# 16lemoing/ccvs

Hardware: AMD Instinct MI355X
Metric: synthesized frames/sec (BAIR 256x256, cond=1, pred=15), whole job (higher is better)
Workload: dtype f32 (convolutions as split-bf16 x3 on bf16 MFMA, fp32 accumulate)

## Files before the change

ccvs_amd/csrc/conv2d_bf16.hip:

```cpp
#include "common.h"
#include "conv_common.h"
#include <stdlib.h>
#include <string.h>
#include <stdio.h>

#define CB_DECL(TWv, MBv) int ccvs_conv_bf16_launch_##TWv##_##MBv(const ConvK& k, const void* wsplit, const void* wktail, int CinG, int halo_h, int halo_w, int ntx_max, int gz, hipStream_t st, int wpc2);
CB_DECL(32, 4) CB_DECL(32, 2) CB_DECL(32, 1) CB_DECL(16, 4) CB_DECL(16, 2) CB_DECL(16, 1) CB_DECL(8, 4) CB_DECL(8, 2) CB_DECL(8, 1)
#undef CB_DECL

extern "C" int ccvs_conv_fetch_bytes_per_lane(const char* kernel_name) {
    if (!kernel_name) return -1;
    const char* pc = strstr(kernel_name, "conv2d_bf16x3_pc_kernel<");
    if (pc) {
        int tw = 0, mb = 0, nty = 0;
        if (sscanf(pc + strlen("conv2d_bf16x3_pc_kernel<"), " %d , %d , %d", &tw, &mb, &nty) != 3) return -1;
        const int b = conv_nty_fetch_bytes(nty);
        return b ? b : -1;
    }
    if (strstr(kernel_name, "conv2d_bf16x3_pt_kernel<")) return 16;
    if (strstr(kernel_name, "conv2d_bf16x3_kernel<") || strstr(kernel_name, "conv2d_mfma_kernel")) return 4;
    return -1;
}

static int g_conv_pt_mode = 1;
extern "C" int ccvs_conv_persistent_tiles(int32_t mode) {
    const int prev = __atomic_exchange_n(&g_conv_pt_mode, mode < 0 ? __atomic_load_n(&g_conv_pt_mode, __ATOMIC_RELAXED) : (int)(mode & 3), __ATOMIC_RELAXED);
    return prev;
}

extern "C" int ccvs_conv2d_bf16x3(const float* x, const void* w_split, const float* bias, const float* residual, float* y,
                                  const ccvs_conv_desc* d, void* stream) {
    CCVS_REQUIRE(x && w_split && y && d, "ccvs_conv2d_bf16x3: null pointer");
    CCVS_REQUIRE(d->N > 0 && d->Cin > 0 && d->Cout > 0 && d->Hin > 0 && d->Win > 0, "ccvs_conv2d_bf16x3: empty tensor");
    CCVS_REQUIRE((d->kh == d->kw || d->kw == 1 || d->kh == 1) && d->kh >= 1 && d->kh <= 9 && d->kw >= 1 && d->kw <= 9,
                 "ccvs_conv2d_bf16x3: kernel %dx%d unsupported", d->kh, d->kw);
    CCVS_REQUIRE(d->CoutPad % 32 == 0 && d->CoutPad >= d->Cout, "ccvs_conv2d_bf16x3: CoutPad %d invalid for Cout %d", d->CoutPad, d->Cout);
    int Hout, Wout;
    if (d->transposed) {
        CCVS_REQUIRE(d->kh == 3 && d->stride == 2 && d->pad == 0, "ccvs_conv2d_bf16x3: transposed supports k3 s2 p0 only");
        Hout = 2 * d->Hin + d->kh - 2;
        Wout = 2 * d->Win + d->kw - 2;
    } else {
        CCVS_REQUIRE(d->stride == 1 || d->stride == 2, "ccvs_conv2d_bf16x3: stride %d unsupported", d->stride);
        Hout = (d->Hin + 2 * d->pad - d->kh) / d->stride + 1;
        Wout = (d->Win + 2 * d->pad - d->kw) / d->stride + 1;
    }
    CCVS_REQUIRE(Hout == d->Hout && Wout == d->Wout, "ccvs_conv2d_bf16x3: output %dx%d expected, got %dx%d", Hout, Wout, d->Hout, d->Wout);

    ConvK k;
    k.x = x; k.w = nullptr; k.bias = bias; k.res = residual; k.y = y;
    k.N = d->N; k.Cin = d->Cin; k.Hin = d->Hin; k.Win = d->Win; k.in_sN = d->in_sN; k.in_sC = d->in_sC;
    k.Cout = d->Cout; k.CoutPad = d->CoutPad; k.Hout = d->Hout; k.Wout = d->Wout;
    k.out_sN = d->out_sN; k.out_sC = d->out_sC; k.res_sN = d->res_sN; k.res_sC = d->res_sC;
    k.kh = d->kh; k.kw = d->kw; k.stride = d->stride; k.pad = d->pad; k.transposed = d->transposed ? 1 : 0;
    k.act = d->act; k.accumulate = d->accumulate; k.out_scale = d->out_scale;
    k.pre = d->pre; k.pre_sN = d->pre_sN; k.pre_sC = d->pre_sC; k.pre_div = d->pre_div > 0 ? d->pre_div : 1;
    k.in_p8 = d->in_p8 ? 1 : 0; k.out_p8 = d->out_p8 ? 1 : 0;
    static const int pt_env = getenv_int("CCVS_CONV_PT", -1);
    k.pt = pt_env >= 0 ? pt_env : __atomic_load_n(&g_conv_pt_mode, __ATOMIC_RELAXED);
    k.ktail = 0; k.nwork = 0; k.gx = k.gy = 1; k.work0 = 0; k.xcd_chunk = 0; k.cu_limit = d->cu_limit > 0 ? d->cu_limit : ccvs_cu_limit_of(stream);
    k.zi = (d->pre && k.pre_div > 1 && !d->transposed && d->N % k.pre_div == 0) ? k.pre_div : 0;
    if (k.in_p8) CCVS_REQUIRE(!d->transposed && d->stride == 1 && d->Cin % 8 == 0, "ccvs_conv2d_bf16x3: packed input needs stride 1, Cin %% 8 == 0");
    if (k.out_p8) CCVS_REQUIRE(!d->transposed && d->Cout % 8 == 0 && !d->accumulate && !residual, "ccvs_conv2d_bf16x3: packed output needs Cout %% 8 == 0, no residual / accumulate");
    const int CinG = 2 * ((d->Cin + 15) / 16);

    const int VH = d->transposed ? (Hout + 1) / 2 : Hout;
    const int VW = d->transposed ? (Wout + 1) / 2 : Wout;
    const int TW = VW > 16 ? 32 : (VW > 8 ? 16 : 8);
    const int TH = 256 / TW;
    k.tiles_x = cdiv(VW, TW);
    k.tiles_y = cdiv(VH, TH);
    const int s = d->transposed ? 1 : d->stride;
    const int ext_y = d->transposed ? 1 : d->kh - 1, ext_x = d->transposed ? 1 : d->kw - 1;
    const int ntx_max = d->transposed ? 2 : d->kw;
    const int halo_h = (TH - 1) * s + ext_y + 1, halo_w = (TW - 1) * s + ext_x + 1;
    const int gz = d->N * (d->transposed ? 4 : 1);
    CCVS_REQUIRE(gz <= 65535, "ccvs_conv2d_bf16x3: batch %d too large for one launch", d->N);
    hipStream_t st = (hipStream_t)stream;
    int mb = (d->CoutPad % 128 == 0) ? 4 : ((d->CoutPad % 64 == 0) ? 2 : 1);
    constexpr long small_split = 256;
    while (mb > 1 && (long)k.tiles_x * k.tiles_y * gz * (d->CoutPad / (32 * mb)) < small_split) mb >>= 1;
    constexpr int wpc2_cin = 64;
    int wpc2 = 0;
    if (mb >= 2 && TW == 32 && d->Cin <= wpc2_cin && d->kh == 3 && d->kw == 3 && d->stride == 1 && !d->transposed && !d->in_p8 && !d->out_p8) {
        mb = 2;
        wpc2 = 1;
    }
#define CB_DISPATCH(TWv)                                                                                        \
    if (mb == 4) return ccvs_conv_bf16_launch_##TWv##_4(k, w_split, d->w_ktail, CinG, halo_h, halo_w, ntx_max, gz, st, wpc2);           \
    if (mb == 2) return ccvs_conv_bf16_launch_##TWv##_2(k, w_split, d->w_ktail, CinG, halo_h, halo_w, ntx_max, gz, st, wpc2);           \
    return ccvs_conv_bf16_launch_##TWv##_1(k, w_split, d->w_ktail, CinG, halo_h, halo_w, ntx_max, gz, st, wpc2);
    if (TW == 32) { CB_DISPATCH(32) }
    if (TW == 16) { CB_DISPATCH(16) }
    CB_DISPATCH(8)
#undef CB_DISPATCH
}
```

ccvs_amd/csrc/conv2d_bf16_core.h:

```cpp
#pragma once
#include "common.h"
#include "conv_common.h"

typedef __bf16 bf16x8 __attribute__((ext_vector_type(8)));
__device__ __forceinline__ void cb_store16(void* dst, f32x4 v) { *reinterpret_cast<f32x4*>(dst) = v; }
__device__ __forceinline__ void cb_store16(void* dst, uint4 v) { cb_store16(dst, f32x4{__uint_as_float(v.x), __uint_as_float(v.y), __uint_as_float(v.z), __uint_as_float(v.w)}); }

#define CB_NO_CLAMP(c) (c)
#define CB_LDS_BARRIER() asm volatile("s_waitcnt lgkmcnt(0)\n\ts_barrier" ::: "memory")

#define CB_TAP4_PRIME(OFF)                                                                                             \
    {                                                                                                                  \
        _Pragma("unroll") for (int pp = 0; pp < 4; ++pp) {                                                             \
            fq[pp][0] = __builtin_bit_cast(bf16x8, it0[OFF(0) + bofs[pp]]);                                            \
            fq[pp][1] = __builtin_bit_cast(bf16x8, it0[OFF(0) + plane + bofs[pp]]);                                    \
        }                                                                                                              \
        _Pragma("unroll") for (int m = 0; m < MB; ++m) {                                                               \
            fw[0][m][0] = __builtin_bit_cast(bf16x8, wt0[m * 32]);                                                     \
            fw[0][m][1] = __builtin_bit_cast(bf16x8, wt0[NT + m * 32]);                                                \
        }                                                                                                              \
    }
#define CB_TAP4(CUR, tb, more, OFF)                                                                                    \
    {                                                                                                                  \
        const uint4* itn_ = it0 + OFF((tb) + 1);                                                                       \
        if (more) {                                                                                                    \
            const uint4* wtn_ = wt0 + ((tb) + 1) * 4 * NT;                                                             \
            _Pragma("unroll") for (int m = 0; m < MB; ++m) {                                                           \
                fw[(CUR) ^ 1][m][0] = __builtin_bit_cast(bf16x8, wtn_[m * 32]);                                        \
                fw[(CUR) ^ 1][m][1] = __builtin_bit_cast(bf16x8, wtn_[NT + m * 32]);                                   \
            }                                                                                                          \
        }                                                                                                              \
        __builtin_amdgcn_sched_barrier(0);                                                                             \
        _Pragma("unroll") for (int m = 0; m < MB; ++m) {                                                               \
            _Pragma("unroll") for (int pp = 0; pp < 4; ++pp) {                                                         \
                acc[m][pp] = __builtin_amdgcn_mfma_f32_32x32x16_bf16(fw[CUR][m][1], fq[pp][0], acc[m][pp], 0, 0, 0);   \
                acc[m][pp] = __builtin_amdgcn_mfma_f32_32x32x16_bf16(fw[CUR][m][0], fq[pp][1], acc[m][pp], 0, 0, 0);   \
                acc[m][pp] = __builtin_amdgcn_mfma_f32_32x32x16_bf16(fw[CUR][m][0], fq[pp][0], acc[m][pp], 0, 0, 0);   \
                if (m == MB - 1 && (more)) {                                                                           \
                    fq[pp][0] = __builtin_bit_cast(bf16x8, itn_[bofs[pp]]);                                            \
                    fq[pp][1] = __builtin_bit_cast(bf16x8, itn_[plane + bofs[pp]]);                                    \
                }                                                                                                      \
            }                                                                                                          \
        }                                                                                                              \
    }

#define CB_LD_B(SET, tb, OFF)                                                                   \
    {                                                                                           \
        const uint4* it_ = it0 + OFF(tb);                                                       \
        _Pragma("unroll") for (int pp = 0; pp < 2; ++pp) {                                      \
            fb[SET][pp][0] = __builtin_bit_cast(bf16x8, it_[bofs[pp]]);                         \
            fb[SET][pp][1] = __builtin_bit_cast(bf16x8, it_[plane + bofs[pp]]);                 \
        }                                                                                       \
    }
#define CB_LD_A(SET, tb, m_)                                                                    \
    {                                                                                           \
        const uint4* wt_ = wt0 + (tb) * 4 * NT + (m_) * 32;                                     \
        fa[SET][0] = __builtin_bit_cast(bf16x8, wt_[0]);                                        \
        fa[SET][1] = __builtin_bit_cast(bf16x8, wt_[NT]);                                       \
    }
#define CB_TAP(BSET, A0, tb, has_next, OFF)                                                     \
    _Pragma("unroll") for (int m = 0; m < MB; ++m) {                                            \
        if (m + 1 < MB) {                                                                       \
            CB_LD_A(((A0) + m + 1) & 1, tb, m + 1)                                              \
        } else if (has_next) {                                                                  \
            CB_LD_A(((A0) + m + 1) & 1, (tb) + 1, 0)                                            \
            CB_LD_B((BSET) ^ 1, (tb) + 1, OFF)                                                  \
        }                                                                                       \
        __builtin_amdgcn_sched_barrier(0);  \
        _Pragma("unroll") for (int pp = 0; pp < 2; ++pp) {                                      \
            acc[m][pp] = __builtin_amdgcn_mfma_f32_32x32x16_bf16(fa[((A0) + m) & 1][1], fb[BSET][pp][0], acc[m][pp], 0, 0, 0); \
            acc[m][pp] = __builtin_amdgcn_mfma_f32_32x32x16_bf16(fa[((A0) + m) & 1][0], fb[BSET][pp][1], acc[m][pp], 0, 0, 0); \
            acc[m][pp] = __builtin_amdgcn_mfma_f32_32x32x16_bf16(fa[((A0) + m) & 1][0], fb[BSET][pp][0], acc[m][pp], 0, 0, 0); \
        }                                                                                       \
    }

#define CB_KTAIL(IH, WTL)                                                                                              \
    {                                                                                                                  \
        const int r_ = p.ktail, nq_ = 9 * r_, nj_ = (nq_ + 15) >> 4;                                                   \
        const unsigned short* ih = IH;                                                                                 \
        const uint4* wtl = WTL;                                                                                        \
        for (int j = 0; j < nj_; ++j) {                                                                                \
            bf16x8 gb[PP][2];                                                                                          \
            _Pragma("unroll") for (int pp = 0; pp < PP; ++pp) {                                                        \
                unsigned hw[4], lw[4];                                                                                 \
                _Pragma("unroll") for (int i = 0; i < 8; ++i) {                                                        \
                    const int q = 16 * j + 8 * khalf + i;                                                              \
                    const int qc = min(q, nq_ - 1);                                                                    \
                    const int t = qc / r_, c = qc - t * r_;                                                            \
                    const int tyy = t / 3, txx = t - 3 * tyy;                                                          \
                    const int e = (bofs[pp] + tyy * IWS + txx) * 8 + c;    \
                    unsigned hv = ih[e], lv = ih[plane * 8 + e];                                                       \
                    if (q >= nq_) { hv = 0; lv = 0; }                                                                  \
                    if (i & 1) { hw[i >> 1] |= hv << 16; lw[i >> 1] |= lv << 16; }                                     \
                    else { hw[i >> 1] = hv; lw[i >> 1] = lv; }                                                         \
                }                                                                                                      \
                gb[pp][0] = __builtin_bit_cast(bf16x8, make_uint4(hw[0], hw[1], hw[2], hw[3]));                        \
                gb[pp][1] = __builtin_bit_cast(bf16x8, make_uint4(lw[0], lw[1], lw[2], lw[3]));                        \
            }                                                                                                          \
            _Pragma("unroll") for (int m = 0; m < MB; ++m) {                                                           \
                const bf16x8 ah = __builtin_bit_cast(bf16x8, wtl[j * 4 * NT + m * 32]);                                \
                const bf16x8 al = __builtin_bit_cast(bf16x8, wtl[j * 4 * NT + NT + m * 32]);                           \
                _Pragma("unroll") for (int pp = 0; pp < PP; ++pp) {                                                    \
                    acc[m][pp] = __builtin_amdgcn_mfma_f32_32x32x16_bf16(al, gb[pp][0], acc[m][pp], 0, 0, 0);          \
                    acc[m][pp] = __builtin_amdgcn_mfma_f32_32x32x16_bf16(ah, gb[pp][1], acc[m][pp], 0, 0, 0);          \
                    acc[m][pp] = __builtin_amdgcn_mfma_f32_32x32x16_bf16(ah, gb[pp][0], acc[m][pp], 0, 0, 0);          \
                }                                                                                                      \
            }                                                                                                          \
        }                                                                                                              \
    }

#define CB_STAGE_PASS(ACC, P8, RW, LANE, KHALF)                                                                        \
    if (P8) {                                                                                                          \
        _Pragma("unroll") for (int pp = 0; pp < PP; ++pp) {                                                            \
            float* sp = stage + (((RW) * PP + pp) * 32 + ((LANE) & 31)) * 36 + 4 * (KHALF);                            \
            _Pragma("unroll") for (int g = 0; g < 4; ++g) {                                                            \
                const f32x4 q4 = {ACC[pp][4 * g], ACC[pp][4 * g + 1], ACC[pp][4 * g + 2], ACC[pp][4 * g + 3]};         \
                *reinterpret_cast<f32x4*>(sp + 8 * g) = q4;                                                            \
            }                                                                                                          \
        }                                                                                                              \
    } else {                                                                                                           \
        _Pragma("unroll") for (int pp = 0; pp < PP; ++pp)                                                              \
            _Pragma("unroll") for (int r = 0; r < 16; ++r)                                                             \
                stage[((r & 3) + 8 * (r >> 2) + 4 * (KHALF)) * NPIX + ((RW) * PP + pp) * 32 + ((LANE) & 31)] = ACC[pp][r]; \
    }

#define CB_EPI_OFFS(i, TID, STRIDE)                                                                  \
// ... 75 lines not shown
```

ccvs_amd/csrc/conv2d_bf16_kernels.h:

```cpp
#pragma once
#include "common.h"
#include "conv_common.h"
#include "conv2d_bf16_core.h"
#include <stdlib.h>
#include <stdio.h>

typedef unsigned u32x4 __attribute__((ext_vector_type(4)));

#define CB_CC 16
#define CB_MAX_E 5

typedef __attribute__((address_space(3))) void lds_void;
typedef __attribute__((address_space(1))) const void glb_void;

static __device__ uint4 g_conv_zero16 = {0u, 0u, 0u, 0u};

__device__ __forceinline__ void stage_pixel(const float* __restrict__ xn, long in_sC, int Cin, int c0, int off, uint4* in_tile, int plane,
                                            int e) {
    const bool inside = off >= 0;
    const float* src = xn + (inside ? off : 0);
    const bool full = (c0 + CB_CC <= Cin);
#pragma unroll
    for (int h = 0; h < 2; ++h) {
        float v[8];
// ... 152 lines not shown
                    bh[pp] = __builtin_bit_cast(bf16x8, it[bofs[pp]]);
                    bl[pp] = __builtin_bit_cast(bf16x8, it[plane + bofs[pp]]);
                }
#pragma unroll
                for (int m = 0; m < MB; ++m) {
                    const bf16x8 ah = __builtin_bit_cast(bf16x8, wt[m * 32]);
                    const bf16x8 al = __builtin_bit_cast(bf16x8, wt[NT + m * 32]);
#pragma unroll
                    for (int pp = 0; pp < PP; ++pp) {
                        acc[m][pp] = __builtin_amdgcn_mfma_f32_32x32x16_bf16(al, bh[pp], acc[m][pp], 0, 0, 0);
                        acc[m][pp] = __builtin_amdgcn_mfma_f32_32x32x16_bf16(ah, bl[pp], acc[m][pp], 0, 0, 0);
                        acc[m][pp] = __builtin_amdgcn_mfma_f32_32x32x16_bf16(ah, bh[pp], acc[m][pp], 0, 0, 0);
                    }
                }
            }
        }
    }

    const int add_kind = conv_add_kind(p);
#pragma unroll
    for (int pp = 0; pp < PP; ++pp) {
        const int pj = (wave * PP + pp) * 32 + (lane & 31);
        const int prow = pj / TW, pcol = pj - prow * TW;
        const int vy = ty * TH + prow, vx = tx * TW + pcol;
        if (vy >= ay.V || vx >= ax.V) continue;
        const int oy = vy * ay.os + ay.oo, ox = vx * ax.os + ax.oo;
        const long opix = (long)oy * p.Wout + ox;
#pragma unroll
        for (int m = 0; m < MB; ++m) {
            if constexpr (MB == 1) {
#pragma unroll
                for (int r = 0; r < 16; ++r) {
                    const int co = n0 + m * 32 + (r & 3) + 8 * (r >> 2) + 4 * khalf;
                    if (co < p.Cout) {
                        float v = acc[m][pp][r];
                        if (p.pre) v += p.pre[(long)(n / p.pre_div) * p.pre_sN + (long)co * p.pre_sC + opix];
                        if (p.bias) v += p.bias[co];
                        if (p.act == CCVS_ACT_LRELU) v = lrelu01(v);
                        if (p.res) v += p.res[(long)n * p.res_sN + (long)co * p.res_sC + opix];
                        v *= p.out_scale;
                        float* dst = p.y + (long)n * p.out_sN + (long)co * p.out_sC + opix;
                        if (p.accumulate) v += *dst;
                        *dst = v;
                    }
                }
            } else {
                epi_block16(p, acc[m][pp], bias_s + m * 32 + 4 * khalf, n, n0 + m * 32 + 4 * khalf, opix, add_kind);
            }
        }
    }
}

#define CB_PC_OFF(tb) (xd0 + (tb) * xdd)
template <int TW, int MB, int NTY, int PP = 2, int WPC = 1>
__global__ __launch_bounds__(512, ((MB == 1 && PP == 2) || WPC == 2) ? 4 : 2) void conv2d_bf16x3_pc_kernel(ConvK p, const uint4* __restrict__ wsplit, int CinG, int ntx_max) {
    static_assert(WPC == 1 || (WPC == 2 && MB == 2 && PP == 2 && NTY == 3), "two workgroups per CU: the 64-channel 3 x 3 form only");
    static_assert(PP == 2 || (PP == 4 && (NTY > 0 || NTY == -83) && MB == 2), "the 512-pixel tile exists for the VEC / packed staging modes and 64 output channels");
    static_assert(conv_nty_fetch_bytes(NTY) != 0, "unknown staging mode: classify it in conv_common.h (conv_nty_*)");
    constexpr bool VEC = conv_nty_vec(NTY);
    constexpr bool P8IN = conv_nty_p8(NTY);
    constexpr bool TAP3 = NTY == 3 || NTY == -83;
    constexpr bool DMAW = VEC || P8IN;
    constexpr int CB_XQ = (NTY == -2) ? 2 : 1;
    constexpr int NPIX = 128 * PP;
    constexpr int TH = NPIX / TW;
    constexpr int NT = 32 * MB;
    constexpr int NP = 256;
    constexpr int NPW = 256;
    constexpr int NPX = 256;
    constexpr int NTXM = (MB == 1) ? 9 : 3;
    constexpr int CB_WR = (NTXM * 4 * NT + NPW - 1) / NPW;
    extern __shared__ __attribute__((aligned(16))) uint4 smem4[];
    __shared__ float bias_s[32 * MB];

    const int tid = threadIdx.x, lane = tid & 63, wave = tid >> 6;
    const bool producer = wave >= 4;
    const int rt = producer ? tid - 256 : tid, rw = wave & 3;
    const bool xrole = VEC && producer;
    const int rtw = rt;
    CONV_TILE_COORDS(p, bx, by, bz)
    const int ty = bx / p.tiles_x, tx = bx - ty * p.tiles_x;
    const int n0 = by * NT;
    const int n = bz;
    constexpr bool GEO3 = TAP3;
    const AxisTaps ay = GEO3 ? axis_taps_k3(p.Hout) : axis_taps(p.kh, p.stride, p.pad, 0, 0, p.Hout);
    const AxisTaps ax = GEO3 ? axis_taps_k3(p.Wout) : axis_taps(p.kw, p.stride, p.pad, 0, 0, p.Wout);
    if (ty * TH >= ay.V || tx * TW >= ax.V) return;
    if (tid < 32 * MB) bias_s[tid] = (p.bias && n0 + tid < p.Cout) ? p.bias[n0 + tid] : 0.f;

    const int IH = (TH - 1) * ay.s + ay.ext + 1;
    const int IW = (TW - 1) * ax.s + ax.ext + 1;
    const int iy0 = ty * TH * ay.s + ay.lo, ix0 = tx * TW * ax.s + ax.lo;
    const int xsh = VEC ? ((ax.lo % 4) + 4) % 4 : 0;
    const int NQ = (xsh + IW + 3) >> 2;
    const int IWS = VEC ? 4 * NQ + 1 : IW;
    const int plane = IH * IWS;
    const int ntxm_ = GEO3 ? 3 : ntx_max;
    const int in_sz = 4 * plane, w_sz = ntxm_ * 4 * NT;
    uint4* in_buf = smem4;
    uint4* w_buf = smem4 + 2 * in_sz;

    const float* xn = p.x + (long)n * p.in_sN;
    const int nt = ay.nt;
    const int nchunks = (p.Cin + CB_CC - 1) / CB_CC;
    const bool ktail = NTY == 3 && p.ktail > 0;
    const int nsteps = ktail ? (nchunks - 1) * nt + 1 : nchunks * nt;
    const int wunits = ax.nt * 4 * NT;

    constexpr int NE = (VEC || P8IN) ? 1 : CB_MAX_E;
    int offs[NE];
    {
        int er = 0, ec = 0;
        const int dr_ = NP / IW, dc_ = NP - dr_ * IW;
        if (!VEC && !P8IN && producer) { er = rt / IW; ec = rt - er * IW; }
#pragma unroll
        for (int j = 0; j < NE; ++j) {
            const int e = rt + NP * j;
            offs[j] = -2;
            if (!VEC && !P8IN && producer && e < plane) {
                const int gy = iy0 + er, gx = ix0 + ec;
                offs[j] = (gy >= 0 && gy < p.Hin && gx >= 0 && gx < p.Win) ? gy * p.Win + gx : -1;
            }
            er += dr_; ec += dc_;
            if (ec >= IW) { ec -= IW; ++er; }
        }
    }
    auto pix_offset = [&](int j) -> int {
        int o = -2;
#pragma unroll
        for (int jj = 0; jj < NE; ++jj) o = (j == jj) ? offs[jj] : o;
        return o;
    };
    constexpr int NI = PP / 2;
    bool vitem[NI], vin[NI];
    int ve[NI], vh[NI];
    const float* vptr[NI];
#pragma unroll
    for (int j = 0; j < NI; ++j) { vitem[j] = false; vin[j] = false; ve[j] = 0; vh[j] = 0; vptr[j] = xn; }
    if (xrole) {
        const int NQP = (NQ + 1) >> 1;
        const int per_half = NQP * IH * 2;
        const int n_items = per_half * 2;
#pragma unroll
        for (int j = 0; j < NI; ++j) {
            const int it0_ = rt + NPX * j;
            const int it = min(it0_, n_items - 1);
            vh[j] = it / per_half;
            const int rem = it - vh[j] * per_half;
            const int t = rem >> 1;
            const int qh = t / IH;
            const int vr = t - qh * IH;
            int vq = 2 * qh + (rem & 1);
            vitem[j] = it0_ < n_items && vq < NQ;
            vq = min(vq, NQ - 1);
            const int gy = iy0 + vr, gxa = ix0 - xsh + 4 * vq;
            vin[j] = gy >= 0 && gy < p.Hin && gxa >= 0 && gxa < p.Win;
            vptr[j] = xn + (long)(8 * vh[j]) * p.in_sC + (vin[j] ? gy * p.Win + gxa : 0);
            ve[j] = vr * IWS + 4 * vq;
        }
    }
    f32x4 xv[2][NI][VEC ? 8 : 1];
    int xvc0[2] = {-1, -1};
    int wofs[CB_WR];
#pragma unroll
    for (int i = 0; i < CB_WR; ++i) {
        const int ic = min(rtw + NPW * i, wunits - 1);
        const int b = ic / (4 * NT), rem = ic - b * (4 * NT);
        const int hp = rem / NT, co = rem - hp * NT;
        wofs[i] = ((b * ax.dw * CinG + (hp >> 1)) * 2 + (hp & 1)) * p.CoutPad + co;
    }
    u32x4 wraw[CB_WR];
    float xraw[CB_XQ][VEC ? 1 : 16];
    int xoff[CB_XQ], xc0 = 0;
#pragma unroll
    for (int q = 0; q < CB_XQ; ++q) xoff[q] = -2;

    const int ay_w0 = ay.w0, ay_dw = ay.dw, ax_w0 = ax.w0, kw_ = p.kw, cout_pad = p.CoutPad, cin_ = p.Cin;
    const long in_sC = p.in_sC;
    auto load_w = [&](int ci_, int a_) {
        const uint4* base = wsplit + ((((long)(ay_w0 + a_ * ay_dw) * kw_ + ax_w0) * CinG + ci_ * 2) * 2) * cout_pad + n0;
#pragma unroll
        for (int i = 0; i < CB_WR; ++i) wraw[i] = *reinterpret_cast<const u32x4*>(base + wofs[i]);
    };
    auto store_w = [&](uint4* dst) {
#pragma unroll
        for (int i = 0; i < CB_WR; ++i)
// ... 50 lines not shown
        xvc0[set] = c_ * CB_CC;
        const bool full = xvc0[set] + CB_CC <= cin_;
#pragma unroll
        for (int j = 0; j < NI; ++j) {
#pragma unroll
            for (int i = 0; i < (VEC ? 8 : 1); ++i) {
                const int c = full ? xvc0[set] + i : min(xvc0[set] + 8 * vh[j] + i, cin_ - 1) - 8 * vh[j];
                xv[set][j][i] = *reinterpret_cast<const f32x4*>(vptr[j] + (long)c * in_sC);
            }
        }
    };
    auto store_xv = [&](int set, uint4* dst) {
        if (xvc0[set] < 0) return;
#pragma unroll
        for (int j = 0; j < NI; ++j) {
            if (!vitem[j]) continue;
            const bool plain = vin[j] && (xvc0[set] + CB_CC <= cin_);
#pragma unroll
            for (int px = 0; px < 4; ++px) {
                float v[8];
#pragma unroll
                for (int i = 0; i < 8; ++i) v[i] = xv[set][j][VEC ? i : 0][px];
                if (!plain) {
#pragma unroll
                    for (int i = 0; i < 8; ++i) v[i] = (vin[j] && xvc0[set] + 8 * vh[j] + i < cin_) ? v[i] : 0.f;
                }
                uint4 hi, lo;
                split8(v, hi, lo);
                dst[(vh[j] * 2 + 0) * plane + ve[j] + px] = hi;
                dst[(vh[j] * 2 + 1) * plane + ve[j] + px] = lo;
            }
        }
    };
    auto load_x = [&](int c_, int slot) {
        xc0 = c_ * CB_CC;
        const bool full = (xc0 + CB_CC <= cin_);
#pragma unroll
        for (int q = 0; q < CB_XQ; ++q) {
            xoff[q] = pix_offset(slot + q * nt);
            if (xoff[q] != -2) {
                const int o = max(xoff[q], 0);
#pragma unroll
                for (int i = 0; i < (VEC ? 1 : 16); ++i) {
                    const float* cb = xn + (long)(full ? xc0 + i : min(xc0 + i, cin_ - 1)) * in_sC;
                    xraw[q][i] = cb[o];
                }
            }
        }
    };
    auto store_x = [&](int slot, uint4* dst) {
#pragma unroll
        for (int q = 0; q < CB_XQ; ++q) {
            if (xoff[q] == -2) continue;
            const int e = rt + NP * (slot + q * nt);
            const bool plain = (xoff[q] >= 0) && (xc0 + CB_CC <= cin_);
#pragma unroll
            for (int h = 0; h < 2; ++h) {
                float v[8];
#pragma unroll
                for (int i = 0; i < 8; ++i) v[i] = xraw[q][VEC ? 0 : 8 * h + i];
                if (!plain) {
#pragma unroll
                    for (int i = 0; i < 8; ++i) v[i] = (xoff[q] >= 0 && xc0 + 8 * h + i < cin_) ? v[i] : 0.f;
                }
                uint4 hi, lo;
                split8(v, hi, lo);
                dst[(h * 2 + 0) * plane + e] = hi;
                dst[(h * 2 + 1) * plane + e] = lo;
            }
        }
    };

    int bofs[PP];
#pragma unroll
    for (int pp = 0; pp < PP; ++pp) {
        const int pj = (rw * PP + pp) * 32 + (lane & 31);
        const int prow = pj / TW, pcol = pj - prow * TW;
        bofs[pp] = prow * ay.s * IWS + pcol * ax.s + xsh;
    }
    const int khalf = lane >> 5;
    f32x16 acc[MB][PP];
#pragma unroll
    for (int m = 0; m < MB; ++m)
#pragma unroll
        for (int pp = 0; pp < PP; ++pp)
#pragma unroll
            for (int r = 0; r < 16; ++r) acc[m][pp][r] = 0.f;

    if (producer) {
        if (P8IN) {
            dma_x(0, in_buf);
            asm volatile("s_waitcnt vmcnt(0)" ::: "memory");
        } else if (xrole) {
            load_xv(0, 0);
            store_xv(0, in_buf);
        } else if (!VEC) {
            for (int j = 0; j < NE; ++j) {
                const int o = pix_offset(j);
                if (o != -2) stage_pixel(xn, p.in_sC, p.Cin, 0, o, in_buf, plane, rt + NP * j);
            }
        }
        if (!DMAW) {
            const uint4* base = wsplit + ((((long)ay_w0 * kw_ + ax_w0) * CinG) * 2) * cout_pad + n0;
#pragma unroll
            for (int i = 0; i < CB_WR; ++i)
                if (rtw + NPW * i < wunits) w_buf[rtw + NPW * i] = base[wofs[i]];
        }
    }

    if (producer && P8IN) {
        __builtin_amdgcn_s_barrier();
        for (int ci = 0; ci < nchunks; ++ci) {
            for (int a = 0; a < nt; ++a) {
                if (a == 0 && ci + 1 < nchunks) dma_x(ci + 1, in_buf + ((ci + 1) & 1) * in_sz);
                if (a == nt - 1) asm volatile("s_waitcnt vmcnt(0)" ::: "memory");
                __builtin_amdgcn_s_barrier();
            }
        }
    } else if (producer && VEC) {
        constexpr int NTYc = VEC ? NTY : 1;
        constexpr bool deep = WPC == 1;
        load_xv(0, min(1, nchunks - 1));
        if (deep) load_xv(1, min(2, nchunks - 1));
        __syncthreads();
        for (int ci = 0; ci < nchunks; ci += 2) {
            if (ci + 1 < nchunks) store_xv(0, in_buf + ((ci + 1) & 1) * in_sz);
            if (deep) load_xv(0, min(ci + 3, nchunks - 1));
            else load_xv(1, min(ci + 2, nchunks - 1));
#pragma unroll
            for (int a = 0; a < NTYc; ++a) {
                if (a > 0 && ktail && ci == nchunks - 1) break;
                CB_LDS_BARRIER();
            }
            if (ci + 1 >= nchunks) break;
            if (ci + 2 < nchunks) store_xv(1, in_buf + ((ci + 2) & 1) * in_sz);
            if (deep) load_xv(1, min(ci + 4, nchunks - 1));
            else load_xv(0, min(ci + 3, nchunks - 1));
#pragma unroll
            for (int a = 0; a < NTYc; ++a) {
                if (a > 0 && ktail && ci + 1 == nchunks - 1) break;
                CB_LDS_BARRIER();
            }
        }
        asm volatile("s_waitcnt vmcnt(0)" ::: "memory");
    } else if (producer) {
      int ci = -1, a = nt - 1;
      for (int s = -1; s < nsteps; ++s) {
        if (s >= 0) {
            if (s + 1 < nsteps) store_w(w_buf + ((s + 1) & 1) * w_sz);
            if (ci + 1 < nchunks) store_x(a, in_buf + ((ci + 1) & 1) * in_sz);
        }
        int a1 = a + 1, c1 = ci;
        if (a1 == nt) { a1 = 0; ++c1; }
        int a2 = a1 + 1, c2 = c1;
        if (a2 == nt) { a2 = 0; ++c2; }
        if (s + 2 < nsteps) load_w(c2, a2);
        const int cx = (a1 == 0) ? ci + 2 : ci + 1;
        if (cx < nchunks) {
            load_x(cx, a1);
        } else {
#pragma unroll
            for (int q = 0; q < CB_XQ; ++q) xoff[q] = -2;
        }
        __syncthreads();
        if (++a == nt) { a = 0; ++ci; }
      }
    } else {
      int ci = -1, a = nt - 1;
      const int nloop = ktail ? nsteps - 1 : nsteps;
      for (int s = -1; s < nloop; ++s) {
        if (DMAW && s + 1 < nsteps) {
            int a1 = a + 1, c1 = ci;
            if (a1 == nt) { a1 = 0; ++c1; }
            dma_w(c1, a1, w_buf + ((s + 1) & 1) * w_sz);
        }
        if (s >= 0) {
            const uint4* it0 = in_buf + (ci & 1) * in_sz + (khalf * 2) * plane + (ay.d0 + a * ay.dd - ay.lo) * IWS;
            const uint4* wt0 = w_buf + (s & 1) * w_sz + (khalf * 2) * NT + (lane & 31);
            if constexpr (PP == 4) {
                const int ntx = ax.nt, xd0 = ax.d0 - ax.lo, xdd = ax.dd;
                bf16x8 fq[4][2], fw[2][MB][2];
                CB_TAP4_PRIME(CB_PC_OFF)
                if constexpr (TAP3) {
                    CB_TAP4(0, 0, true, CB_PC_OFF)
                    CB_TAP4(1, 1, true, CB_PC_OFF)
                    CB_TAP4(0, 2, false, CB_PC_OFF)
                } else {
                    int tb = 0;
                    for (; tb + 2 <= ntx; tb += 2) {
                        CB_TAP4(0, tb, true, CB_PC_OFF)
                        CB_TAP4(1, tb + 1, (tb + 2 < ntx), CB_PC_OFF)
                    }
                    if (tb < ntx) { CB_TAP4(0, tb, false, CB_PC_OFF) }
                }
            } else if constexpr (WPC == 2) {
                const int ntx = ax.nt, xd0 = ax.d0 - ax.lo, xdd = ax.dd;
#pragma unroll
                for (int tb = 0; tb < 3; ++tb) {
                    if (tb < ntx) {
                        const uint4* it_ = it0 + (xd0 + tb * xdd);
                        const uint4* wt_ = wt0 + tb * 4 * NT;
                        bf16x8 qb[2][2], wa[2][2];
#pragma unroll
                        for (int pp = 0; pp < 2; ++pp) {
                            qb[pp][0] = __builtin_bit_cast(bf16x8, it_[bofs[pp]]);
                            qb[pp][1] = __builtin_bit_cast(bf16x8, it_[plane + bofs[pp]]);
                        }
                        wa[0][0] = __builtin_bit_cast(bf16x8, wt_[0]);
                        wa[0][1] = __builtin_bit_cast(bf16x8, wt_[NT]);
#pragma unroll
                        for (int m = 0; m < MB; ++m) {
                            if (m + 1 < MB) {
                                wa[(m + 1) & 1][0] = __builtin_bit_cast(bf16x8, wt_[(m + 1) * 32]);
                                wa[(m + 1) & 1][1] = __builtin_bit_cast(bf16x8, wt_[NT + (m + 1) * 32]);
                            }
#pragma unroll
                            for (int pp = 0; pp < 2; ++pp) {
                                acc[m][pp] = __builtin_amdgcn_mfma_f32_32x32x16_bf16(wa[m & 1][1], qb[pp][0], acc[m][pp], 0, 0, 0);
                                acc[m][pp] = __builtin_amdgcn_mfma_f32_32x32x16_bf16(wa[m & 1][0], qb[pp][1], acc[m][pp], 0, 0, 0);
                                acc[m][pp] = __builtin_amdgcn_mfma_f32_32x32x16_bf16(wa[m & 1][0], qb[pp][0], acc[m][pp], 0, 0, 0);
                            }
                        }
                    }
                }
            } else {
            bf16x8 fa[2][2];
            bf16x8 fb[2][2][2];
            const int ntx = ax.nt, xd0 = ax.d0 - ax.lo, xdd = ax.dd;
            CB_LD_B(0, 0, CB_PC_OFF)
            CB_LD_A(0, 0, 0)
            if constexpr (TAP3) {
                CB_TAP(0, 0, 0, true, CB_PC_OFF)
// ... 209 lines not shown

template <int TW, int MB>
static int launch_conv_bf16(const ConvK& k_in, const void* wsplit, const void* wktail, int CinG, int halo_h, int halo_w, int ntx_max, int gz, hipStream_t st, int wpc2) {
    constexpr int NT = 32 * MB;
    int plane = halo_h * halo_w;
    const size_t p8s2 = k_in.out_p8 ? (size_t)256 * 36 * 4 : 0, p8s4 = k_in.out_p8 ? (size_t)512 * 36 * 4 : 0;
    if (plane > 256 * CB_MAX_E) {
        ccvs_set_error("ccvs_conv2d_bf16x3: halo tile %dx%d too large", halo_h, halo_w);
        return CCVS_ERR_ARG;
    }
    ConvK k = k_in;
    if constexpr (TW == 32 && (MB == 4 || MB == 2)) {
        const int pt_on = k.pt;
        if (pt_on) {
            const int r = conv_pt_try<MB>(k, wsplit, wktail, CinG, gz, st, pt_on);
            if (r != CONV_PT_NOT_TAKEN) return r;
        }
    }
    const dim3 grid3(k.tiles_x * k.tiles_y, k.CoutPad / NT, gz);
    long n_chunk = 1, cap = 0, total = 0;
    auto plan = [&](const dim3& grid, const void* fn, size_t smem_bytes) {
        total = (long)grid.x * grid.y * grid.z;
        k.nwork = 0; k.work0 = 0;
        k.gx = (int)grid.x; k.gy = (int)grid.y;
        k.xcd_chunk = conv_xcd_chunk(total);
        n_chunk = 1;
        if (k.cu_limit <= 0) return;
        cap = (long)k.cu_limit * conv_occupancy(fn, 512, smem_bytes);
        if (total <= cap) return;
        cap -= cap % 8;
        if (cap < 8) cap = 8;
        k.nwork = (int)total;
        n_chunk = (total + cap - 1) / cap;
    };
    auto chunk_grid = [&](const dim3& grid, long c) -> dim3 {
        if (k.nwork == 0) return grid;
        k.work0 = (int)(c * cap);
        const long n = (total - c * cap < cap) ? total - c * cap : cap;
        k.xcd_chunk = conv_xcd_chunk(n);
        return dim3((unsigned)n);
    };
#define CB_LAUNCH_RETURN_ON(GRID, KERNEL, SMEM, ...)                                                      \
    do {                                                                                          \
        CB_SET_LDS_ONCE(KERNEL, 159 * 1024);                                                      \
        plan(GRID, (const void*)KERNEL, SMEM);                                                    \
        for (long c_ = 0; c_ < n_chunk; ++c_) {                                                   \
            const dim3 g_ = chunk_grid(GRID, c_);                                                 \
            hipLaunchKernelGGL((KERNEL), g_, dim3(512), SMEM, st, k, __VA_ARGS__);                \
        }                                                                                         \
        CCVS_CHECK_LAUNCH("ccvs_conv2d_bf16x3");                                                  \
        return CCVS_OK;                                                                           \
    } while (0)
#define CB_LAUNCH_RETURN(KERNEL, SMEM, ...) CB_LAUNCH_RETURN_ON(grid3, KERNEL, SMEM, __VA_ARGS__)
    if (k.in_p8) {
        const size_t smem_p = (size_t)(2 * 4 * plane + 2 * ntx_max * 4 * NT) * 16;
        if (4 * plane > 8 * 256 || ntx_max > (MB == 1 ? 9 : 3) || smem_p > 156 * 1024) {
            ccvs_set_error("ccvs_conv2d_bf16x3: packed input with a %dx%d halo tile / %d taps per row is not supported", halo_h, halo_w, ntx_max);
            return CCVS_ERR_ARG;
        }
        if constexpr (TW == 32 && MB == 2) {
            const int th4 = 16, halo_h4 = (th4 - 1) + k.kh, plane4 = halo_h4 * halo_w;
            const size_t smem_4 = (size_t)(2 * 4 * plane4 + 2 * ntx_max * 4 * NT) * 16;
            if (k.out_p8 && k.kh == 3 && k.kw == 3 && k.pad == 1 && k.cu_limit <= 0 && k.Hout >= 2 * th4 && 4 * plane4 <= 10 * 256 && smem_4 <= 156 * 1024 &&
                smem_4 >= (size_t)32 * 512 * 4) {
                k.tiles_y = cdiv(k.Hout, th4);
                const dim3 grid4(k.tiles_x * k.tiles_y, k.CoutPad / NT, gz);
                CB_LAUNCH_RETURN_ON(grid4, (conv2d_bf16x3_pc_kernel<TW, MB, -83, 4>), (smem_4 > p8s4 ? smem_4 : p8s4), (const uint4*)wsplit, CinG, ntx_max);
            }
        }
        const size_t smem_p2 = smem_p > p8s2 ? smem_p : p8s2;
        if constexpr (MB != 4) {
            if (k.kh == 3 && k.kw == 3 && k.pad == 1) {
                CB_LAUNCH_RETURN((conv2d_bf16x3_pc_kernel<TW, MB, -83>), smem_p2, (const uint4*)wsplit, CinG, ntx_max);
            }
        }
        CB_LAUNCH_RETURN((conv2d_bf16x3_pc_kernel<TW, MB, -8>), smem_p2, (const uint4*)wsplit, CinG, ntx_max);
    }
    const int xsh = ((-k.pad % 4) + 4) % 4, nq = (xsh + halo_w + 3) / 4;
    const bool vec_ok = !k.transposed && k.stride == 1 && k.Win % 4 == 0 && k.in_sC % 4 == 0 && k.in_sN % 4 == 0 &&
                        (reinterpret_cast<uintptr_t>(k.x) & 15) == 0 && TW >= 16 && halo_h * ((nq + 1) / 2) * 4 <= 256 && ntx_max <= (MB == 1 ? 9 : 3) &&
                        (k.kh == 1 || (k.kh == 3 && k.kw == 3 && k.pad == 1));
    const int ktail_r = k.Cin % CB_CC;
    const bool kt = wktail && vec_ok && k.kh == 3 && k.kw == 3 && ktail_r >= 1 && ktail_r <= 3 && k.Cin > CB_CC;
    if constexpr (TW == 32 && MB == 2) {
        const int th4 = 16, halo_h4 = (th4 - 1) + k.kh;
        const size_t smem_4 = (size_t)(2 * 4 * halo_h4 * (nq * 4 + 1) + 2 * ntx_max * 4 * NT) * 16;
        if (!wpc2 && vec_ok && !k.out_p8 && k.Hout >= 2 * th4 && halo_h4 * ((nq + 1) / 2) * 4 <= 512 && smem_4 <= 156 * 1024 && smem_4 >= (size_t)32 * 512 * 4) {
            k.tiles_y = cdiv(k.Hout, th4);
            const dim3 grid4(k.tiles_x * k.tiles_y, k.CoutPad / NT, gz);
            if (k.cu_limit <= 0) {
                k.ktail = kt ? ktail_r : 0;
                if (k.kh == 3) CB_LAUNCH_RETURN_ON(grid4, (conv2d_bf16x3_pc_kernel<TW, MB, 3, 4>), smem_4, (const uint4*)(kt ? wktail : wsplit), CinG, ntx_max);
                else CB_LAUNCH_RETURN_ON(grid4, (conv2d_bf16x3_pc_kernel<TW, MB, 1, 4>), smem_4, (const uint4*)wsplit, CinG, ntx_max);
            }
            k.tiles_y = k_in.tiles_y;
        }
    }
    if (vec_ok) {
        const size_t smem_v = (size_t)(2 * 4 * halo_h * (nq * 4 + 1) + 2 * ntx_max * 4 * NT) * 16;
        if constexpr (TW == 32 && MB == 2) {
            if (wpc2 && k.kh == 3 && k.kw == 3 && smem_v <= 80 * 1024 && k.cu_limit <= 0) {
                k.ktail = kt ? ktail_r : 0;
                CB_LAUNCH_RETURN((conv2d_bf16x3_pc_kernel<TW, MB, 3, 2, 2>), (smem_v > p8s2 ? smem_v : p8s2), (const uint4*)(kt ? wktail : wsplit), CinG, ntx_max);
            }
        }
        if (smem_v <= 156 * 1024) {
// ... 29 lines not shown
```

ccvs_amd/lib.py:

```python
import ctypes as C
import os

_HERE = os.path.dirname(os.path.abspath(__file__))
LIB_PATH = os.environ.get("CCVS_LIB") or os.path.join(_HERE, "csrc", "libccvs_hip.so")

EXPORTS = [
    "ccvs_last_error", "ccvs_abi_version", "ccvs_conv2d", "ccvs_conv2d_bf16x3", "ccvs_conv_fetch_bytes_per_lane", "ccvs_conv_persistent_tiles", "ccvs_upfirdn2d", "ccvs_dwconvT4x4s2",
    "ccvs_correlation7x7", "ccvs_backwarp", "ccvs_backwarp_ctx", "ccvs_backwarp_p8_ctx", "ccvs_backwarp_proj_ctx", "ccvs_warp_fuse_blend", "ccvs_warp_fuse_blend_ctx", "ccvs_tap_shift_add", "ccvs_vq_argmin", "ccvs_embed_gather", "ccvs_l2_normalize_channels",
    "ccvs_gpt_embed", "ccvs_layernorm", "ccvs_gemm_workspace_bytes", "ccvs_gemm_nt", "ccvs_gemm_ln", "ccvs_gemm_ln_qkv", "ccvs_attention", "ccvs_kv_append", "ccvs_sample_topk", "ccvs_sample_topk_philox", "ccvs_sample_topn",
    "ccvs_gpt_decode_step", "ccvs_gpt_decode_status", "ccvs_gpt_program_bytes", "ccvs_gpt_decode_prepare", "ccvs_pack_u8", "ccvs_pack_u8_norm", "ccvs_stream_cu_limit", "ccvs_psnr", "ccvs_ssim_workspace_bytes", "ccvs_ssim", "ccvs_resize_bilinear",
    "ccvs_deform_conv3x3_ctx", "ccvs_gconvT4x4s2", "ccvs_flow_mask_toff", "ccvs_gaussian_blur", "ccvs_to_rgb", "ccvs_channel_head", "ccvs_mse",
]


class ConvDesc(C.Structure):
    _fields_ = [
        ("N", C.c_int32), ("Cin", C.c_int32), ("Hin", C.c_int32), ("Win", C.c_int32),
        ("in_sN", C.c_int64), ("in_sC", C.c_int64),
        ("Cout", C.c_int32), ("CoutPad", C.c_int32), ("Hout", C.c_int32), ("Wout", C.c_int32),
        ("out_sN", C.c_int64), ("out_sC", C.c_int64), ("res_sN", C.c_int64), ("res_sC", C.c_int64),
        ("kh", C.c_int32), ("kw", C.c_int32), ("stride", C.c_int32), ("pad", C.c_int32), ("transposed", C.c_int32),
        ("act", C.c_int32), ("accumulate", C.c_int32), ("out_scale", C.c_float),
        ("pre", C.c_void_p), ("pre_sN", C.c_int64), ("pre_sC", C.c_int64), ("pre_div", C.c_int32),
        ("in_p8", C.c_int32), ("out_p8", C.c_int32), ("cu_limit", C.c_int32),
        ("w_ktail", C.c_void_p),
    ]


MAX_CTX = 16


class CtxList(C.Structure):
    _fields_ = [("k", C.c_int32), ("p", C.c_void_p * MAX_CTX), ("sN", C.c_int64 * MAX_CTX)]


class GptLayer(C.Structure):
    _fields_ = [(n, C.c_void_p) for n in ("qkv_w", "qkv_b", "qkv_s", "proj_w", "proj_b", "fc_w", "fc_b", "fc_s", "fc2_w", "fc2_b",
                                          "kcache", "vcache")]


class GptDecode(C.Structure):
    _fields_ = [
        ("B", C.c_int32), ("C", C.c_int32), ("H", C.c_int32), ("F", C.c_int32), ("n_layer", C.c_int32), ("Tmax", C.c_int32),
        ("vocab", C.c_int32), ("V", C.c_int32), ("ln_eps", C.c_float),
        ("layers", C.POINTER(GptLayer)),
        ("tok_emb", C.c_void_p), ("pos_table", C.c_void_p), ("pos_off", C.c_int32),
        ("head_w", C.c_void_p), ("head_b", C.c_void_p), ("head_s", C.c_void_p),
        ("tok", C.c_void_p), ("codes", C.c_void_p), ("codes_sB", C.c_int64),
        ("widx", C.c_void_p), ("len", C.c_void_p),
        ("x", C.c_void_p), ("q", C.c_void_p), ("att", C.c_void_p), ("h", C.c_void_p), ("logits", C.c_void_p),
        ("noise", C.c_void_p), ("rng", C.c_int32), ("top_k", C.c_int32), ("temperature", C.c_float),
        ("workspace", C.c_void_p), ("state", C.c_void_p), ("groups", C.c_int32),
        ("noise_stream", C.c_void_p),
        ("persistent", C.c_int32), ("program", C.c_void_p),
    ]


class CcvsError(RuntimeError):
    pass

# ... 82 lines not shown
```

include/ccvs_hip.h:

```cpp
#ifndef CCVS_HIP_H
#define CCVS_HIP_H

#include <stdint.h>

#ifdef __cplusplus
extern "C" {
#endif

#define CCVS_OK 0
#define CCVS_ERR_ARG (-1)
#define CCVS_ERR_LAUNCH (-2)

#define CCVS_ACT_NONE 0
#define CCVS_ACT_LRELU 1

const char* ccvs_last_error(void);
int ccvs_abi_version(void);

typedef struct ccvs_conv_desc {
    int32_t N, Cin, Hin, Win;
    int64_t in_sN, in_sC;
    int32_t Cout, CoutPad, Hout, Wout;
    int64_t out_sN, out_sC;
    int64_t res_sN, res_sC;
    int32_t kh, kw, stride, pad, transposed;
    int32_t act, accumulate;
    float out_scale;
    const float* pre;
    int64_t pre_sN, pre_sC;
    int32_t pre_div;
    int32_t in_p8, out_p8;
    int32_t cu_limit;
    const void* w_ktail;
} ccvs_conv_desc;

int ccvs_conv2d(const float* x, const float* w_packed, const float* bias, const float* residual, float* y,
                const ccvs_conv_desc* d, void* stream);

int ccvs_conv2d_bf16x3(const float* x, const void* w_split, const float* bias, const float* residual, float* y,
                       const ccvs_conv_desc* d, void* stream);

int ccvs_conv_fetch_bytes_per_lane(const char* kernel_name);

int ccvs_conv_persistent_tiles(int32_t mode);

int ccvs_upfirdn2d(const float* x, float* y, const float* residual, int64_t NC, int32_t H, int32_t W, int32_t up,
                   int32_t down, int32_t pad0, int32_t pad1, float gain, int32_t act, float out_scale, void* stream);

int ccvs_dwconvT4x4s2(const float* x, int64_t x_sN, const float* w, float* y, int64_t y_sN, int32_t N, int32_t C, int32_t H,
                      int32_t W, void* stream);

int ccvs_gaussian_blur(const float* x, int64_t x_sN, int64_t x_sC, float* y, int32_t N, int32_t C, int32_t H, int32_t W, int32_t k,
                       const float* weights, void* stream);

int ccvs_to_rgb(const float* x, int64_t x_sN, const float* w, const float* b_conv, const float* bias, const float* skip, float* y,
                int32_t N, int32_t C, int32_t H, int32_t W, void* stream);

int ccvs_channel_head(const float* x, int64_t x_sN, const float* w, float scale, const float* bias, float* y, int32_t N, int32_t C,
                      int32_t H, int32_t W, int32_t act, int32_t tanh_out, void* stream);

int ccvs_correlation7x7(const float* first, const float* second, float* out, int32_t N, int32_t C, int32_t H, int32_t W,
                        int32_t stride, int32_t first_div, int32_t lrelu, void* stream);

int ccvs_backwarp(const float* x, int64_t x_sN, int64_t x_sC, const float* flow, int64_t flow_sN, float flow_mult, float* y,
                  int64_t y_sN, int64_t y_sC, int32_t N, int32_t C, int32_t H, int32_t W, void* stream);

#define CCVS_MAX_CTX 16
typedef struct ccvs_ctx_list {
    int32_t k;
    const float* p[CCVS_MAX_CTX];
    int64_t sN[CCVS_MAX_CTX];
} ccvs_ctx_list;
int ccvs_backwarp_ctx(const ccvs_ctx_list* ctx, int64_t x_sC, const float* flow, int64_t flow_sN, float flow_mult, float* y,
                      int64_t y_sN, int64_t y_sC, int32_t N, int32_t C, int32_t H, int32_t W, void* stream);
int ccvs_warp_fuse_blend_ctx(float* dec, int64_t dec_sN, int64_t dec_sC, const ccvs_ctx_list* ctx, const float* flows,
                             int64_t flows_sN, const float* occs, int64_t occs_sN, float flow_mult, int32_t N, int32_t C,
                             int32_t H, int32_t W, void* stream);

int ccvs_backwarp_p8_ctx(const ccvs_ctx_list* ctx, int64_t x_sC, const float* flow_occ, int64_t fo_sN, float flow_mult, void* y_p8,
                         int32_t N, int32_t C, int32_t H, int32_t W, void* stream);

int ccvs_backwarp_proj_ctx(const ccvs_ctx_list* ctx, int64_t x_sC, const float* flow, int64_t flow_sN, float flow_mult,
                           const float* w_t, const float* bias, float* y, int32_t N, int32_t Cin, int32_t Cout, int32_t CoutPad,
                           int32_t H, int32_t W, int32_t act, void* stream);

int ccvs_warp_fuse_blend(float* dec, int64_t dec_sN, int64_t dec_sC, const float* ctx, const float* flows, int64_t flows_sN,
                         const float* occs, int64_t occs_sN, float flow_mult, int32_t N, int32_t k, int32_t C, int32_t H,
                         int32_t W, void* stream);

int ccvs_tap_shift_add(const float* t, const float* bias, float* y, int64_t y_sN, int32_t N, int32_t k, int32_t H, int32_t W,
                       int32_t accumulate, int32_t vertical, void* stream);

int ccvs_vq_argmin(const float* z, const float* codebook_t, const float* e_sq, int64_t* idx, int32_t N, int32_t C, int32_t HW,
                   int32_t n_e, void* stream);

// ... 97 lines not shown
```

Measured before the change: 202.7.

## Add stride-2 3x3 conv path with parity-split LDS staging and 128-pixel tiles

```diff
diff --git a/ccvs_amd/csrc/conv2d_bf16.hip b/ccvs_amd/csrc/conv2d_bf16.hip
--- a/ccvs_amd/csrc/conv2d_bf16.hip
+++ b/ccvs_amd/csrc/conv2d_bf16.hip
@@ -27,6 +27,9 @@
     const int prev = __atomic_exchange_n(&g_conv_pt_mode, mode < 0 ? __atomic_load_n(&g_conv_pt_mode, __ATOMIC_RELAXED) : (int)(mode & 3), __ATOMIC_RELAXED);
     return prev;
 }
+
+static int g_conv_s2_pc_launches = 0;
+extern "C" int ccvs_conv_s2_pc_launches(void) { return __atomic_load_n(&g_conv_s2_pc_launches, __ATOMIC_RELAXED); }
 
 extern "C" int ccvs_conv2d_bf16x3(const float* x, const void* w_split, const float* bias, const float* residual, float* y,
                                   const ccvs_conv_desc* d, void* stream) {
@@ -67,7 +70,9 @@
     const int VH = d->transposed ? (Hout + 1) / 2 : Hout;
     const int VW = d->transposed ? (Wout + 1) / 2 : Wout;
     const int TW = VW > 16 ? 32 : (VW > 8 ? 16 : 8);
-    const int TH = 256 / TW;
+    static const int s2_env = getenv_int("CCVS_CONV_S2_PC", 1);
+    const bool s2pc = s2_env && !d->transposed && d->stride == 2 && d->kh == 3 && d->kw == 3 && !d->out_p8;
+    const int TH = (s2pc ? 128 : 256) / TW;
     k.tiles_x = cdiv(VW, TW);
     k.tiles_y = cdiv(VH, TH);
     const int s = d->transposed ? 1 : d->stride;
@@ -81,7 +86,8 @@
     constexpr long small_split = 256;
     while (mb > 1 && (long)k.tiles_x * k.tiles_y * gz * (d->CoutPad / (32 * mb)) < small_split) mb >>= 1;
     constexpr int wpc2_cin = 64;
-    int wpc2 = 0;
+    if (s2pc) __atomic_fetch_add(&g_conv_s2_pc_launches, 1, __ATOMIC_RELAXED);
+    int wpc2 = s2pc ? 2 : 0;
     if (mb >= 2 && TW == 32 && d->Cin <= wpc2_cin && d->kh == 3 && d->kw == 3 && d->stride == 1 && !d->transposed && !d->in_p8 && !d->out_p8) {
         mb = 2;
         wpc2 = 1;
diff --git a/ccvs_amd/csrc/conv2d_bf16_core.h b/ccvs_amd/csrc/conv2d_bf16_core.h
--- a/ccvs_amd/csrc/conv2d_bf16_core.h
+++ b/ccvs_amd/csrc/conv2d_bf16_core.h
@@ -72,6 +72,28 @@
             acc[m][pp] = __builtin_amdgcn_mfma_f32_32x32x16_bf16(fa[((A0) + m) & 1][0], fb[BSET][pp][1], acc[m][pp], 0, 0, 0); \
             acc[m][pp] = __builtin_amdgcn_mfma_f32_32x32x16_bf16(fa[((A0) + m) & 1][0], fb[BSET][pp][0], acc[m][pp], 0, 0, 0); \
         }                                                                                       \
+    }
+
+#define CB_LD1(SET, tb, OFF)                                                                                           \
+    {                                                                                                                  \
+        const uint4* it_ = it0 + OFF(tb);                                                                              \
+        const uint4* wt_ = wt0 + (tb) * 4 * NT;                                                                        \
+        fq[SET][0] = __builtin_bit_cast(bf16x8, it_[bofs[0]]);                                                         \
+        fq[SET][1] = __builtin_bit_cast(bf16x8, it_[plane + bofs[0]]);                                                 \
+        _Pragma("unroll") for (int m = 0; m < MB; ++m) {                                                               \
+            fw[SET][m][0] = __builtin_bit_cast(bf16x8, wt_[m * 32]);                                                   \
+            fw[SET][m][1] = __builtin_bit_cast(bf16x8, wt_[NT + m * 32]);                                              \
+        }                                                                                                              \
+    }
+#define CB_TAP1(CUR, tb, more, OFF)                                                                                    \
+    {                                                                                                                  \
+        if (more) { CB_LD1((CUR) ^ 1, (tb) + 1, OFF) }                                                                 \
+        __builtin_amdgcn_sched_barrier(0);                                                                             \
+        _Pragma("unroll") for (int m = 0; m < MB; ++m) {                                                               \
+            acc[m][0] = __builtin_amdgcn_mfma_f32_32x32x16_bf16(fw[CUR][m][1], fq[CUR][0], acc[m][0], 0, 0, 0);        \
+            acc[m][0] = __builtin_amdgcn_mfma_f32_32x32x16_bf16(fw[CUR][m][0], fq[CUR][1], acc[m][0], 0, 0, 0);        \
+            acc[m][0] = __builtin_amdgcn_mfma_f32_32x32x16_bf16(fw[CUR][m][0], fq[CUR][0], acc[m][0], 0, 0, 0);        \
+        }                                                                                                              \
     }
 
 #define CB_KTAIL(IH, WTL)                                                                                              \
diff --git a/ccvs_amd/csrc/conv2d_bf16_kernels.h b/ccvs_amd/csrc/conv2d_bf16_kernels.h
--- a/ccvs_amd/csrc/conv2d_bf16_kernels.h
+++ b/ccvs_amd/csrc/conv2d_bf16_kernels.h
@@ -228,10 +228,13 @@
 }
 
 #define CB_PC_OFF(tb) (xd0 + (tb) * xdd)
-template <int TW, int MB, int NTY, int PP = 2, int WPC = 1>
+#define CB_S2_OD(TW) ((TW) + 4)
+#define CB_S2_OFF(tb) (((tb) & 1) * CB_S2_OD(TW) + ((tb) >> 1))
+template <int TW, int MB, int NTY, int PP = 2, int WPC = 1, int S = 1>
 __global__ __launch_bounds__(512, ((MB == 1 && PP == 2) || WPC == 2) ? 4 : 2) void conv2d_bf16x3_pc_kernel(ConvK p, const uint4* __restrict__ wsplit, int CinG, int ntx_max) {
+    static_assert((S == 1 && PP != 1) || (S == 2 && PP == 1 && NTY == 0 && WPC == 1), "stride 2: the 128-pixel tile with scalar staging, and nothing else uses that tile");
     static_assert(WPC == 1 || (WPC == 2 && MB == 2 && PP == 2 && NTY == 3), "two workgroups per CU: the 64-channel 3 x 3 form only");
-    static_assert(PP == 2 || (PP == 4 && (NTY > 0 || NTY == -83) && MB == 2), "the 512-pixel tile exists for the VEC / packed staging modes and 64 output channels");
+    static_assert(PP <= 2 || (PP == 4 && (NTY > 0 || NTY == -83) && MB == 2), "the 512-pixel tile exists for the VEC / packed staging modes and 64 output channels");
     static_assert(conv_nty_fetch_bytes(NTY) != 0, "unknown staging mode: classify it in conv_common.h (conv_nty_*)");
     constexpr bool VEC = conv_nty_vec(NTY);
     constexpr bool P8IN = conv_nty_p8(NTY);
@@ -269,7 +272,7 @@
     const int iy0 = ty * TH * ay.s + ay.lo, ix0 = tx * TW * ax.s + ax.lo;
     const int xsh = VEC ? ((ax.lo % 4) + 4) % 4 : 0;
     const int NQ = (xsh + IW + 3) >> 2;
-    const int IWS = VEC ? 4 * NQ + 1 : IW;
+    const int IWS = VEC ? 4 * NQ + 1 : (S == 2 ? 2 * TW + 4 : IW);
     const int plane = IH * IWS;
     const int ntxm_ = GEO3 ? 3 : ntx_max;
     const int in_sz = 4 * plane, w_sz = ntxm_ * 4 * NT;
@@ -285,6 +288,11 @@
 
     constexpr int NE = (VEC || P8IN) ? 1 : CB_MAX_E;
     int offs[NE];
+    [[maybe_unused]] int epos[S == 2 ? NE : 1];
+    if constexpr (S == 2) {
+#pragma unroll
+        for (int j = 0; j < NE; ++j) epos[j] = 0;
+    }
     {
         int er = 0, ec = 0;
         const int dr_ = NP / IW, dc_ = NP - dr_ * IW;
@@ -293,9 +301,10 @@
         for (int j = 0; j < NE; ++j) {
             const int e = rt + NP * j;
             offs[j] = -2;
-            if (!VEC && !P8IN && producer && e < plane) {
+            if (!VEC && !P8IN && producer && e < (S == 2 ? IH * IW : plane)) {
                 const int gy = iy0 + er, gx = ix0 + ec;
                 offs[j] = (gy >= 0 && gy < p.Hin && gx >= 0 && gx < p.Win) ? gy * p.Win + gx : -1;
+                if constexpr (S == 2) epos[j] = er * IWS + (ec & 1) * CB_S2_OD(TW) + (ec >> 1);
             }
             er += dr_; ec += dc_;
             if (ec >= IW) { ec -= IW; ++er; }
@@ -307,7 +316,17 @@
         for (int jj = 0; jj < NE; ++jj) o = (j == jj) ? offs[jj] : o;
         return o;
     };
-    constexpr int NI = PP / 2;
+    [[maybe_unused]] auto pix_slot = [&](int j) -> int {
+        if constexpr (S == 2) {
+            int o = 0;
+#pragma unroll
+            for (int jj = 0; jj < NE; ++jj) o = (j == jj) ? epos[jj] : o;
+            return o;
+        } else {
+            return rt + NP * j;
+        }
+    };
+    constexpr int NI = PP >= 2 ? PP / 2 : 1;
     bool vitem[NI], vin[NI];
     int ve[NI], vh[NI];
     const float* vptr[NI];
@@ -464,7 +483,7 @@
 #pragma unroll
         for (int q = 0; q < CB_XQ; ++q) {
             if (xoff[q] == -2) continue;
-            const int e = rt + NP * (slot + q * nt);
+            const int e = S == 2 ? pix_slot(slot + q * nt) : rt + NP * (slot + q * nt);
             const bool plain = (xoff[q] >= 0) && (xc0 + CB_CC <= cin_);
 #pragma unroll
             for (int h = 0; h < 2; ++h) {
@@ -488,7 +507,7 @@
     for (int pp = 0; pp < PP; ++pp) {
         const int pj = (rw * PP + pp) * 32 + (lane & 31);
         const int prow = pj / TW, pcol = pj - prow * TW;
-        bofs[pp] = prow * ay.s * IWS + pcol * ax.s + xsh;
+        bofs[pp] = S == 2 ? prow * 2 * IWS + pcol : prow * ay.s * IWS + pcol * ax.s + xsh;
     }
     const int khalf = lane >> 5;
     f32x16 acc[MB][PP];
@@ -509,7 +528,7 @@
         } else if (!VEC) {
             for (int j = 0; j < NE; ++j) {
                 const int o = pix_offset(j);
-                if (o != -2) stage_pixel(xn, p.in_sC, p.Cin, 0, o, in_buf, plane, rt + NP * j);
+                if (o != -2) stage_pixel(xn, p.in_sC, p.Cin, 0, o, in_buf, plane, S == 2 ? pix_slot(j) : rt + NP * j);
             }
         }
         if (!DMAW) {
@@ -589,7 +608,13 @@
         if (s >= 0) {
             const uint4* it0 = in_buf + (ci & 1) * in_sz + (khalf * 2) * plane + (ay.d0 + a * ay.dd - ay.lo) * IWS;
             const uint4* wt0 = w_buf + (s & 1) * w_sz + (khalf * 2) * NT + (lane & 31);
-            if constexpr (PP == 4) {
+            if constexpr (PP == 1) {
+                bf16x8 fq[2][2], fw[2][MB][2];
+                CB_LD1(0, 0, CB_S2_OFF)
+                CB_TAP1(0, 0, true, CB_S2_OFF)
+                CB_TAP1(1, 1, true, CB_S2_OFF)
+                CB_TAP1(0, 2, false, CB_S2_OFF)
+            } else if constexpr (PP == 4) {
                 const int ntx = ax.nt, xd0 = ax.d0 - ax.lo, xdd = ax.dd;
                 bf16x8 fq[4][2], fw[2][MB][2];
                 CB_TAP4_PRIME(CB_PC_OFF)
@@ -905,6 +930,11 @@
         return CCVS_OK;                                                                           \
     } while (0)
 #define CB_LAUNCH_RETURN(KERNEL, SMEM, ...) CB_LAUNCH_RETURN_ON(grid3, KERNEL, SMEM, __VA_ARGS__)
+    if (wpc2 & 2) {
+        const size_t smem_s2 = (size_t)(2 * 4 * halo_h * (2 * TW + 4) + 2 * 3 * 4 * NT) * 16;
+        CB_LAUNCH_RETURN((conv2d_bf16x3_pc_kernel<TW, MB, 0, 1, 1, 2>), smem_s2, (const uint4*)wsplit, CinG, 3);
+    }
+    wpc2 &= 1;
     if (k.in_p8) {
         const size_t smem_p = (size_t)(2 * 4 * plane + 2 * ntx_max * 4 * NT) * 16;
         if (4 * plane > 8 * 256 || ntx_max > (MB == 1 ? 9 : 3) || smem_p > 156 * 1024) {
diff --git a/ccvs_amd/lib.py b/ccvs_amd/lib.py
--- a/ccvs_amd/lib.py
+++ b/ccvs_amd/lib.py
@@ -5,7 +5,7 @@
 LIB_PATH = os.environ.get("CCVS_LIB") or os.path.join(_HERE, "csrc", "libccvs_hip.so")
 
 EXPORTS = [
-    "ccvs_last_error", "ccvs_abi_version", "ccvs_conv2d", "ccvs_conv2d_bf16x3", "ccvs_conv_fetch_bytes_per_lane", "ccvs_conv_persistent_tiles", "ccvs_upfirdn2d", "ccvs_dwconvT4x4s2",
+    "ccvs_last_error", "ccvs_abi_version", "ccvs_conv2d", "ccvs_conv2d_bf16x3", "ccvs_conv_fetch_bytes_per_lane", "ccvs_conv_s2_pc_launches", "ccvs_conv_persistent_tiles", "ccvs_upfirdn2d", "ccvs_dwconvT4x4s2",
     "ccvs_correlation7x7", "ccvs_backwarp", "ccvs_backwarp_ctx", "ccvs_backwarp_p8_ctx", "ccvs_backwarp_proj_ctx", "ccvs_warp_fuse_blend", "ccvs_warp_fuse_blend_ctx", "ccvs_tap_shift_add", "ccvs_vq_argmin", "ccvs_embed_gather", "ccvs_l2_normalize_channels",
     "ccvs_gpt_embed", "ccvs_layernorm", "ccvs_gemm_workspace_bytes", "ccvs_gemm_nt", "ccvs_gemm_ln", "ccvs_gemm_ln_qkv", "ccvs_attention", "ccvs_kv_append", "ccvs_sample_topk", "ccvs_sample_topk_philox", "ccvs_sample_topn",
     "ccvs_gpt_decode_step", "ccvs_gpt_decode_status", "ccvs_gpt_program_bytes", "ccvs_gpt_decode_prepare", "ccvs_pack_u8", "ccvs_pack_u8_norm", "ccvs_stream_cu_limit", "ccvs_psnr", "ccvs_ssim_workspace_bytes", "ccvs_ssim", "ccvs_resize_bilinear",
diff --git a/include/ccvs_hip.h b/include/ccvs_hip.h
--- a/include/ccvs_hip.h
+++ b/include/ccvs_hip.h
@@ -41,6 +41,8 @@
                        const ccvs_conv_desc* d, void* stream);
 
 int ccvs_conv_fetch_bytes_per_lane(const char* kernel_name);
+
+int ccvs_conv_s2_pc_launches(void);
 
 int ccvs_conv_persistent_tiles(int32_t mode);
 
```

Result: no change. 202.8 (median of 2 runs) (+0.1%).
